# liyheng/MAGPO

Hardware: NVIDIA B200
Metric: end_to_end_training_agent_env_steps_per_sec (higher is better)
Workload: dtype f32

## Files before the change

### magpo_b200/csrc/retention_chunk.cu

```cuda
#include "common.cuh"
#include "kernels.cuh"

namespace magpo {
namespace {

constexpr int RC_ROWS = 32;
constexpr int LDA = 68;
constexpr int LDB = 72;
constexpr int LDP = 36;
constexpr int LDPT = 40;

struct Frag {
  uint32_t h[4], l[4];
};
struct FragB {
  uint32_t h[2], l[2];
};

__device__ __forceinline__ void split(float x, uint32_t& hi, uint32_t& lo) {
  hi = __float_as_uint(x) & 0xFFFFE000u;
  lo = __float_as_uint(x - __uint_as_float(hi));
}

__device__ __forceinline__ void mma8(float (&c)[4], const uint32_t (&a)[4], const uint32_t (&b)[2]) {
  asm volatile(
      "mma.sync.aligned.m16n8k8.row.col.f32.tf32.tf32.f32 {%0,%1,%2,%3}, {%4,%5,%6,%7}, {%8,%9}, {%0,%1,%2,%3};"
      : "+f"(c[0]), "+f"(c[1]), "+f"(c[2]), "+f"(c[3])
      : "r"(a[0]), "r"(a[1]), "r"(a[2]), "r"(a[3]), "r"(b[0]), "r"(b[1]));
}
__device__ __forceinline__ void mma3(float (&c)[4], const Frag& a, const FragB& b) {
  mma8(c, a.l, b.h);
  mma8(c, a.h, b.l);
  mma8(c, a.h, b.h);
}

__device__ __forceinline__ void ldsm_x4(const float* p, uint32_t (&r)[4]) {
  const uint32_t a = (uint32_t)__cvta_generic_to_shared(p);
  asm volatile("ldmatrix.sync.aligned.m8n8.x4.shared.b16 {%0,%1,%2,%3}, [%4];" : "=r"(r[0]), "=r"(r[1]), "=r"(r[2]), "=r"(r[3]) : "r"(a) : "memory");
}
__device__ __forceinline__ void ldsm_x2(const float* p, uint32_t (&r)[2]) {
  const uint32_t a = (uint32_t)__cvta_generic_to_shared(p);
  asm volatile("ldmatrix.sync.aligned.m8n8.x2.shared.b16 {%0,%1}, [%2];" : "=r"(r[0]), "=r"(r[1]) : "r"(a) : "memory");
}
__device__ __forceinline__ void split_u(uint32_t x, uint32_t& hi, uint32_t& lo) {
  hi = x & 0xFFFFE000u;
  lo = __float_as_uint(__uint_as_float(x) - __uint_as_float(hi));
}

__device__ __forceinline__ Frag lda_row(const float* X, int ld, int m0, int k0, int g, int tq) {
  const int lane = 4 * g + tq;
  uint32_t r[4];
  ldsm_x4(X + (m0 + (lane & 7) + ((lane >> 3) & 1) * 8) * ld + k0 + (lane >> 4) * 4, r);
  Frag f;
#pragma unroll
  for (int i = 0; i < 4; ++i) split_u(r[i], f.h[i], f.l[i]);
  return f;
}
__device__ __forceinline__ Frag lda_tr(const float* X, int ld, int m0, int k0, int g, int tq) {
  Frag f;
  split(X[(k0 + tq) * ld + m0 + g], f.h[0], f.l[0]);
  split(X[(k0 + tq) * ld + m0 + g + 8], f.h[1], f.l[1]);
  split(X[(k0 + tq + 4) * ld + m0 + g], f.h[2], f.l[2]);
  split(X[(k0 + tq + 4) * ld + m0 + g + 8], f.h[3], f.l[3]);
  return f;
}
__device__ __forceinline__ FragB ldb(const float* Y, int ld, int k0, int n0, int g, int tq) {
  FragB f;
  split(Y[(k0 + tq) * ld + n0 + g], f.h[0], f.l[0]);
  split(Y[(k0 + tq + 4) * ld + n0 + g], f.h[1], f.l[1]);
  return f;
}
__device__ __forceinline__ FragB ldb_tr(const float* Y, int ld, int k0, int n0, int g, int tq) {
  const int lane = 4 * g + tq;
  uint32_t r[2];
  ldsm_x2(Y + (n0 + (lane & 7)) * ld + k0 + ((lane >> 3) & 1) * 4, r);
  FragB f;
  split_u(r[0], f.h[0], f.l[0]);
  split_u(r[1], f.h[1], f.l[1]);
  return f;
}

__device__ __forceinline__ void zero4(float (&c)[4]) { c[0] = c[1] = c[2] = c[3] = 0.f; }

struct ChunkDecay {
  int cd_lane;
  __device__ __forceinline__ void init(const uint8_t* done, int t0, int L, int N, int n, int lane) {
    const bool d = done && lane < L && done[(int64_t)(t0 + lane) * N + n];
    const unsigned m = __ballot_sync(0xffffffffu, d);
    cd_lane = __popc(m & (0xffffffffu >> (31 - lane)));
  }
  __device__ __forceinline__ int cd(int tl) const { return __shfl_sync(0xffffffffu, cd_lane, tl); }
};

struct Tables {
  float* kpow;
  int* cds;
  uint8_t* row_tl;
};

template <bool CAUSAL>
__device__ __forceinline__ float decay_nm(const Tables& tb, int n, int m) {
  const int tn = tb.row_tl[n], tm = tb.row_tl[m];
  const bool order = CAUSAL ? (n >= m) : (tn >= tm);
  if (!order || tb.cds[tn] != tb.cds[tm]) return 0.f;
  return tb.kpow[tn - tm];
}

template <bool CAUSAL>
__global__ void __launch_bounds__(256, 2)
retention_chunk_fwd_kernel(int T, int N, int A, int Lc, float kappa, const float* __restrict__ q, const float* __restrict__ k,
                           const float* __restrict__ v, int ld, const float* __restrict__ H0, const uint8_t* __restrict__ done,
                           float* __restrict__ ret, float* __restrict__ Hck, float* __restrict__ Hout) {
  extern __shared__ __align__(16) float sm[];
  float* Hp = sm;
  float* Qs = Hp + 64 * LDB;
  float* Ks = Qs + RC_ROWS * LDA;
  float* Kt = Ks + RC_ROWS * LDA;
  float* Vs = Kt + RC_ROWS * LDB;
  float* Ps = Vs + RC_ROWS * LDB;
  Tables tb;
  tb.kpow = Ps + RC_ROWS * LDP;
  tb.cds = reinterpret_cast<int*>(tb.kpow + 40);
  tb.row_tl = reinterpret_cast<uint8_t*>(tb.cds + 32);

  const int n = blockIdx.x, tid = threadIdx.x, warp = tid >> 5, lane = tid & 31, g = lane >> 2, tq = lane & 3;
  if (tid == 0) {
    float p = 1.f;
    for (int j = 0; j < 40; ++j) { tb.kpow[j] = p; p *= kappa; }
  }
  if (tid < 32) tb.row_tl[tid] = (uint8_t)(tid / A);
  for (int i = tid; i < RC_ROWS * LDP; i += 256) Ps[i] = 0.f;

  const int mt = warp & 3, nt0 = (warp >> 2) * 4;
  float Hacc[4][4];
#pragma unroll
  for (int j = 0; j < 4; ++j) {
    const int r = 16 * mt + g, c = 8 * (nt0 + j) + 2 * tq;
    float2 lo2 = make_float2(0.f, 0.f), hi2 = make_float2(0.f, 0.f);
    if (H0) {
      lo2 = *reinterpret_cast<const float2*>(H0 + ((int64_t)n * 64 + r) * 64 + c);
      hi2 = *reinterpret_cast<const float2*>(H0 + ((int64_t)n * 64 + r + 8) * 64 + c);
    }
    Hacc[j][0] = lo2.x; Hacc[j][1] = lo2.y; Hacc[j][2] = hi2.x; Hacc[j][3] = hi2.y;
  }

  const int nchunks = (T + Lc - 1) / Lc;
  float pq[8], pk[8], pv[8];
  auto fetch = [&](int ch) {
    const int t0 = ch * Lc, L = min(Lc, T - t0), rows = L * A;
#pragma unroll
    for (int j = 0; j < 8; ++j) {
      const int idx = tid + j * 256, row = idx >> 6, col = idx & 63;
      pq[j] = pk[j] = pv[j] = 0.f;
      if (row < rows) {
        const int tl = tb.row_tl[row];
        const int64_t grow = ((int64_t)(t0 + tl) * N + n) * A + (row - tl * A);
        pq[j] = q[grow * ld + col]; pk[j] = k[grow * ld + col]; pv[j] = v[grow * ld + col];
      }
    }
  };
  __syncthreads();
  fetch(0);

  for (int ch = 0; ch < nchunks; ++ch) {
    const int t0 = ch * Lc, L = min(Lc, T - t0), rows = L * A;
    ChunkDecay cdk;
    cdk.init(done, t0, L, N, n, lane);
    const int cd_last = cdk.cd(L - 1);
    if (warp == 0) tb.cds[lane] = cdk.cd_lane;
#pragma unroll
    for (int j = 0; j < 4; ++j) {
      const int r = 16 * mt + g, c = 8 * (nt0 + j) + 2 * tq;
      *reinterpret_cast<float2*>(Hp + r * LDB + c) = make_float2(Hacc[j][0], Hacc[j][1]);
      *reinterpret_cast<float2*>(Hp + (r + 8) * LDB + c) = make_float2(Hacc[j][2], Hacc[j][3]);
      if (Hck) {
        float* dst = Hck + (((int64_t)ch * N + n) * 64) * 64;
        *reinterpret_cast<float2*>(dst + r * 64 + c) = make_float2(Hacc[j][0], Hacc[j][1]);
        *reinterpret_cast<float2*>(dst + (r + 8) * 64 + c) = make_float2(Hacc[j][2], Hacc[j][3]);
      }
    }
#pragma unroll
    for (int j = 0; j < 8; ++j) {
      const int idx = tid + j * 256, row = idx >> 6, col = idx & 63;
      const int tl = tb.row_tl[row];
      const int cdt = cdk.cd(tl);
      const float e = (row < rows && cdt == cd_last) ? tb.kpow[L - 1 - tl] : 0.f;
      Qs[row * LDA + col] = pq[j];
      Ks[row * LDA + col] = pk[j];
      Kt[row * LDB + col] = pk[j] * e;
      Vs[row * LDB + col] = pv[j];
    }
    __syncthreads();
    if (ch + 1 < nchunks) fetch(ch + 1);

    float o2[2][4];
    zero4(o2[0]); zero4(o2[1]);
    {
      const int mi = warp >> 2, ni = warp & 3;
      float s[4];
      zero4(s);
#pragma unroll
      for (int k0 = 0; k0 < 64; k0 += 8) {
        const Frag a0 = lda_row(Qs, LDA, 0, k0, g, tq);
        const Frag a1 = lda_row(Qs, LDA, 16, k0, g, tq);
        const FragB bk = ldb_tr(Ks, LDA, k0, 8 * ni, g, tq);
        mma3(s, mi ? a1 : a0, bk);
        const FragB bh = ldb(Hp, LDB, k0, 8 * warp, g, tq);
        mma3(o2[0], a0, bh);
        mma3(o2[1], a1, bh);
      }
      const int r = 16 * mi + g, c = 8 * ni + 2 * tq;
      Ps[r * LDP + c] = s[0] * decay_nm<CAUSAL>(tb, r, c);
      Ps[r * LDP + c + 1] = s[1] * decay_nm<CAUSAL>(tb, r, c + 1);
      Ps[(r + 8) * LDP + c] = s[2] * decay_nm<CAUSAL>(tb, r + 8, c);
      Ps[(r + 8) * LDP + c + 1] = s[3] * decay_nm<CAUSAL>(tb, r + 8, c + 1);
    }
    __syncthreads();

    {
      float o1[2][4];
      zero4(o1[0]); zero4(o1[1]);
#pragma unroll
      for (int k0 = 0; k0 < RC_ROWS; k0 += 8) {
        const FragB bv = ldb(Vs, LDB, k0, 8 * warp, g, tq);
        mma3(o1[0], lda_row(Ps, LDP, 0, k0, g, tq), bv);
        mma3(o1[1], lda_row(Ps, LDP, 16, k0, g, tq), bv);
      }
#pragma unroll
      for (int mi = 0; mi < 2; ++mi)
#pragma unroll
        for (int h = 0; h < 2; ++h) {
          const int row = 16 * mi + g + 8 * h;
          if (row < rows) {
            const int tl = tb.row_tl[row];
            const float cc = (tb.cds[tl] == 0) ? tb.kpow[tl + 1] : 0.f;
            const int64_t grow = ((int64_t)(t0 + tl) * N + n) * A + (row - tl * A);
            *reinterpret_cast<float2*>(ret + grow * 64 + 8 * warp + 2 * tq) =
                make_float2(o1[mi][2 * h] + cc * o2[mi][2 * h], o1[mi][2 * h + 1] + cc * o2[mi][2 * h + 1]);
          }
        }
    }
    {
      const float cL = (cd_last == 0) ? tb.kpow[L] : 0.f;
#pragma unroll
      for (int j = 0; j < 4; ++j)
#pragma unroll
        for (int x = 0; x < 4; ++x) Hacc[j][x] *= cL;
#pragma unroll
      for (int k0 = 0; k0 < RC_ROWS; k0 += 8) {
        const Frag a = lda_tr(Kt, LDB, 16 * mt, k0, g, tq);
#pragma unroll
        for (int j = 0; j < 4; ++j) mma3(Hacc[j], a, ldb(Vs, LDB, k0, 8 * (nt0 + j), g, tq));
      }
    }
    __syncthreads();
  }
  if (Hout) {
#pragma unroll
    for (int j = 0; j < 4; ++j) {
      const int r = 16 * mt + g, c = 8 * (nt0 + j) + 2 * tq;
      float* dst = Hout + (int64_t)n * 64 * 64;
      *reinterpret_cast<float2*>(dst + r * 64 + c) = make_float2(Hacc[j][0], Hacc[j][1]);
      *reinterpret_cast<float2*>(dst + (r + 8) * 64 + c) = make_float2(Hacc[j][2], Hacc[j][3]);
    }
  }
}

template <bool CAUSAL>
__global__ void __launch_bounds__(256, 2)
retention_chunk_bwd_kernel(int T, int N, int A, int Lc, float kappa, const float* __restrict__ q, const float* __restrict__ k,
                           const float* __restrict__ v, int ld, const uint8_t* __restrict__ done,
                           const float* __restrict__ Hck, const float* __restrict__ dret, float* __restrict__ dq,
                           float* __restrict__ dk, float* __restrict__ dv, int ldd) {
  extern __shared__ __align__(16) float sm[];
  float* Hp = sm;
  float* Gs = Hp + 64 * LDA;
  float* Gt = Gs + 64 * LDA;
  float* Qs = Gt + 64 * LDA;
  float* Ks = Qs + RC_ROWS * LDA;
  float* Vs = Ks + RC_ROWS * LDA;
  float* Ds = Vs + RC_ROWS * LDA;
  float* Qc = Ds + RC_ROWS * LDA;
  float* Ps = Qc + RC_ROWS * LDB;
  float* Ws = Ps + RC_ROWS * LDPT;
  Tables tb;
  tb.kpow = Ws + RC_ROWS * LDP;
  tb.cds = reinterpret_cast<int*>(tb.kpow + 40);
  tb.row_tl = reinterpret_cast<uint8_t*>(tb.cds + 32);

  const int n = blockIdx.x, tid = threadIdx.x, warp = tid >> 5, lane = tid & 31, g = lane >> 2, tq = lane & 3;
  if (tid == 0) {
    float p = 1.f;
    for (int j = 0; j < 40; ++j) { tb.kpow[j] = p; p *= kappa; }
  }
  if (tid < 32) tb.row_tl[tid] = (uint8_t)(tid / A);

  const int mt = warp & 3, nt0 = (warp >> 2) * 4;
  float Gacc[4][4];
#pragma unroll
  for (int j = 0; j < 4; ++j) zero4(Gacc[j]);

  const int nchunks = (T + Lc - 1) / Lc;
  float pq[8], pk[8], pv[8], pd[8];
  auto fetch = [&](int ch) {
    const int t0 = ch * Lc, L = min(Lc, T - t0), rows = L * A;
#pragma unroll
    for (int j = 0; j < 8; ++j) {
      const int idx = tid + j * 256, row = idx >> 6, col = idx & 63;
      pq[j] = pk[j] = pv[j] = pd[j] = 0.f;
      if (row < rows) {
        const int tl = tb.row_tl[row];
        const int64_t grow = ((int64_t)(t0 + tl) * N + n) * A + (row - tl * A);
        pq[j] = q[grow * ld + col]; pk[j] = k[grow * ld + col]; pv[j] = v[grow * ld + col];
        pd[j] = dret[grow * 64 + col];
      }
    }
  };
  __syncthreads();
  fetch(nchunks - 1);

  for (int ch = nchunks - 1; ch >= 0; --ch) {
    const int t0 = ch * Lc, L = min(Lc, T - t0), rows = L * A;
    ChunkDecay cdk;
    cdk.init(done, t0, L, N, n, lane);
    const int cd_last = cdk.cd(L - 1);
    if (warp == 0) tb.cds[lane] = cdk.cd_lane;
#pragma unroll
    for (int j = 0; j < 4; ++j) {
      const int r = 16 * mt + g, c = 8 * (nt0 + j) + 2 * tq;
      *reinterpret_cast<float2*>(Gs + r * LDA + c) = make_float2(Gacc[j][0], Gacc[j][1]);
      *reinterpret_cast<float2*>(Gs + (r + 8) * LDA + c) = make_float2(Gacc[j][2], Gacc[j][3]);
      Gt[c * LDA + r] = Gacc[j][0];
      Gt[(c + 1) * LDA + r] = Gacc[j][1];
      Gt[c * LDA + r + 8] = Gacc[j][2];
      Gt[(c + 1) * LDA + r + 8] = Gacc[j][3];
    }
    {
      const float4* src = reinterpret_cast<const float4*>(Hck + ((int64_t)ch * N + n) * 64 * 64);
#pragma unroll
      for (int j = 0; j < 4; ++j) {
        const int idx = tid + j * 256;
        const float4 h = src[idx];
        *reinterpret_cast<float4*>(Hp + (idx >> 4) * LDA + (idx & 15) * 4) = h;
      }
    }
#pragma unroll
    for (int j = 0; j < 8; ++j) {
      const int idx = tid + j * 256, row = idx >> 6, col = idx & 63;
      const int tl = tb.row_tl[row];
      const int cdt = cdk.cd(tl);
      const float cc = (row < rows && cdt == 0) ? tb.kpow[tl + 1] : 0.f;
      Qs[row * LDA + col] = pq[j];
      Ks[row * LDA + col] = pk[j];
      Vs[row * LDA + col] = pv[j];
      Ds[row * LDA + col] = pd[j];
      Qc[row * LDB + col] = pq[j] * cc;
    }
    __syncthreads();
    if (ch > 0) fetch(ch - 1);

    float dq2[2][4], dk2[2][4], dv2[2][4];
    zero4(dq2[0]); zero4(dq2[1]); zero4(dk2[0]); zero4(dk2[1]); zero4(dv2[0]); zero4(dv2[1]);
    {
      const int mi = warp >> 2, ni = warp & 3;
      float s[4], w[4];
      zero4(s); zero4(w);
#pragma unroll
      for (int k0 = 0; k0 < 64; k0 += 8) {
        {
          const Frag a = lda_row(Qs, LDA, 16 * mi, k0, g, tq);
          mma3(s, a, ldb_tr(Ks, LDA, k0, 8 * ni, g, tq));
        }
        const Frag d0 = lda_row(Ds, LDA, 0, k0, g, tq);
        const Frag d1 = lda_row(Ds, LDA, 16, k0, g, tq);
        mma3(w, mi ? d1 : d0, ldb_tr(Vs, LDA, k0, 8 * ni, g, tq));
        {
          const FragB b = ldb_tr(Hp, LDA, k0, 8 * warp, g, tq);
          mma3(dq2[0], d0, b);
          mma3(dq2[1], d1, b);
        }
        {
          const FragB b = ldb_tr(Gs, LDA, k0, 8 * warp, g, tq);
          mma3(dk2[0], lda_row(Vs, LDA, 0, k0, g, tq), b);
          mma3(dk2[1], lda_row(Vs, LDA, 16, k0, g, tq), b);
        }
        {
          const FragB b = ldb_tr(Gt, LDA, k0, 8 * warp, g, tq);
          mma3(dv2[0], lda_row(Ks, LDA, 0, k0, g, tq), b);
          mma3(dv2[1], lda_row(Ks, LDA, 16, k0, g, tq), b);
        }
      }
      const int r = 16 * mi + g, c = 8 * ni + 2 * tq;
      const float d00 = decay_nm<CAUSAL>(tb, r, c), d01 = decay_nm<CAUSAL>(tb, r, c + 1);
      const float d10 = decay_nm<CAUSAL>(tb, r + 8, c), d11 = decay_nm<CAUSAL>(tb, r + 8, c + 1);
      Ps[r * LDPT + c] = s[0] * d00; Ps[r * LDPT + c + 1] = s[1] * d01;
      Ps[(r + 8) * LDPT + c] = s[2] * d10; Ps[(r + 8) * LDPT + c + 1] = s[3] * d11;
      Ws[r * LDP + c] = w[0] * d00; Ws[r * LDP + c + 1] = w[1] * d01;
      Ws[(r + 8) * LDP + c] = w[2] * d10; Ws[(r + 8) * LDP + c + 1] = w[3] * d11;
    }
    __syncthreads();

    {
      float dq1[2][4], dk1[2][4], dv1[2][4];
      zero4(dq1[0]); zero4(dq1[1]); zero4(dk1[0]); zero4(dk1[1]); zero4(dv1[0]); zero4(dv1[1]);
#pragma unroll
      for (int k0 = 0; k0 < RC_ROWS; k0 += 8) {
        {
          const FragB b = ldb(Ks, LDA, k0, 8 * warp, g, tq);
          mma3(dq1[0], lda_row(Ws, LDP, 0, k0, g, tq), b);
          mma3(dq1[1], lda_row(Ws, LDP, 16, k0, g, tq), b);
        }
        {
          const FragB b = ldb(Qs, LDA, k0, 8 * warp, g, tq);
          mma3(dk1[0], lda_tr(Ws, LDP, 0, k0, g, tq), b);
          mma3(dk1[1], lda_tr(Ws, LDP, 16, k0, g, tq), b);
        }
        {
          const FragB b = ldb(Ds, LDA, k0, 8 * warp, g, tq);
          mma3(dv1[0], lda_tr(Ps, LDPT, 0, k0, g, tq), b);
          mma3(dv1[1], lda_tr(Ps, LDPT, 16, k0, g, tq), b);
        }
      }
#pragma unroll
      for (int mi = 0; mi < 2; ++mi)
#pragma unroll
        for (int h = 0; h < 2; ++h) {
          const int row = 16 * mi + g + 8 * h;
          if (row < rows) {
            const int tl = tb.row_tl[row];
            const int cdt = tb.cds[tl];
            const float cc = (cdt == 0) ? tb.kpow[tl + 1] : 0.f;
            const float ee = (cdt == cd_last) ? tb.kpow[L - 1 - tl] : 0.f;
            const int64_t grow = ((int64_t)(t0 + tl) * N + n) * A + (row - tl * A);
            const int col = 8 * warp + 2 * tq;
            *reinterpret_cast<float2*>(dq + grow * ldd + col) =
                make_float2(dq1[mi][2 * h] + cc * dq2[mi][2 * h], dq1[mi][2 * h + 1] + cc * dq2[mi][2 * h + 1]);
            *reinterpret_cast<float2*>(dk + grow * ldd + col) =
                make_float2(dk1[mi][2 * h] + ee * dk2[mi][2 * h], dk1[mi][2 * h + 1] + ee * dk2[mi][2 * h + 1]);
            *reinterpret_cast<float2*>(dv + grow * ldd + col) =
                make_float2(dv1[mi][2 * h] + ee * dv2[mi][2 * h], dv1[mi][2 * h + 1] + ee * dv2[mi][2 * h + 1]);
          }
        }
    }
    {
      const float cL = (cd_last == 0) ? tb.kpow[L] : 0.f;
#pragma unroll
      for (int j = 0; j < 4; ++j)
#pragma unroll
        for (int x = 0; x < 4; ++x) Gacc[j][x] *= cL;
#pragma unroll
      for (int k0 = 0; k0 < RC_ROWS; k0 += 8) {
        const Frag a = lda_tr(Qc, LDB, 16 * mt, k0, g, tq);
#pragma unroll
        for (int j = 0; j < 4; ++j) mma3(Gacc[j], a, ldb(Ds, LDA, k0, 8 * (nt0 + j), g, tq));
      }
    }
    __syncthreads();
  }
}

constexpr size_t kFwdSmem = (size_t)(64 * LDB + 2 * RC_ROWS * LDA + 2 * RC_ROWS * LDB + RC_ROWS * LDP + 40 + 32 + 8) * sizeof(float);
constexpr size_t kBwdSmem =
    (size_t)(3 * 64 * LDA + 4 * RC_ROWS * LDA + RC_ROWS * LDB + RC_ROWS * LDPT + RC_ROWS * LDP + 40 + 32 + 8) * sizeof(float);

template <typename Kern>
int set_smem(Kern kern, size_t bytes) {
  MAGPO_CUDA_OK(cudaFuncSetAttribute(kern, cudaFuncAttributeMaxDynamicSharedMemorySize, (int)bytes));
  return MAGPO_OK;
}

}

int retention_chunk_len(int A) { return std::max(1, RC_ROWS / A); }
int retention_num_chunks(int T, int A) { return (T + retention_chunk_len(A) - 1) / retention_chunk_len(A); }

int retention_chunk_fwd(cudaStream_t s, int T, int N, int A, float kappa, bool causal, const float* q, const float* k,
                        const float* v, int ld, const float* H0, const uint8_t* done, float* ret, float* Hck, float* Hout) {
  const int Lc = retention_chunk_len(A);
  if (once_per_device(ONCE_RET_FWD)) {
    MAGPO_TRY(set_smem(retention_chunk_fwd_kernel<true>, kFwdSmem));
    MAGPO_TRY(set_smem(retention_chunk_fwd_kernel<false>, kFwdSmem));
  }
  ProfScope ps(PROF_RET_FWD, s, 4.0 * 256.0 * (double)T * N * A);
  if (causal)
    retention_chunk_fwd_kernel<true><<<N, 256, kFwdSmem, s>>>(T, N, A, Lc, kappa, q, k, v, ld, H0, done, ret, Hck, Hout);
  else
    retention_chunk_fwd_kernel<false><<<N, 256, kFwdSmem, s>>>(T, N, A, Lc, kappa, q, k, v, ld, H0, done, ret, Hck, Hout);
  MAGPO_LAUNCH_OK();
  return MAGPO_OK;
}

int retention_chunk_bwd(cudaStream_t s, int T, int N, int A, float kappa, bool causal, const float* q, const float* k,
                        const float* v, int ld, const uint8_t* done, const float* Hck, const float* dret, float* dq,
                        float* dk, float* dv, int ldd) {
  const int Lc = retention_chunk_len(A);
  if (once_per_device(ONCE_RET_BWD)) {
    MAGPO_TRY(set_smem(retention_chunk_bwd_kernel<true>, kBwdSmem));
    MAGPO_TRY(set_smem(retention_chunk_bwd_kernel<false>, kBwdSmem));
  }
  ProfScope ps(PROF_RET_BWD, s, 7.0 * 256.0 * (double)T * N * A);
  if (causal)
    retention_chunk_bwd_kernel<true><<<N, 256, kBwdSmem, s>>>(T, N, A, Lc, kappa, q, k, v, ld, done, Hck, dret, dq, dk, dv, ldd);
  else
    retention_chunk_bwd_kernel<false><<<N, 256, kBwdSmem, s>>>(T, N, A, Lc, kappa, q, k, v, ld, done, Hck, dret, dq, dk, dv, ldd);
  MAGPO_LAUNCH_OK();
  return MAGPO_OK;
}

}
```

Baseline: 8.359 million.

## Prefetch chunk state via cp.async and hoist done-flag loads into fetch

In the backward retention kernel, the per-chunk Hck state load changes from synchronous float4 global reads into shared memory to cp.async issued one chunk ahead, right after the sync that follows Hp's last use. It is waited on at the start of the next iteration. The done-flag loads in both forward and backward kernels move into the prefetch lambda so their latency overlaps the previous chunk's compute. The aim is to hide global memory latency on the sequential chunk loop, which adds correctness risk around reuse of the Hp buffer.

```diff
diff --git a/magpo_b200/csrc/retention_chunk.cu b/magpo_b200/csrc/retention_chunk.cu
--- a/magpo_b200/csrc/retention_chunk.cu
+++ b/magpo_b200/csrc/retention_chunk.cu
@@ -80,12 +80,21 @@
   return f;
 }
 
+__device__ __forceinline__ void cp_async16(float* dst, const float* src) {
+  asm volatile("cp.async.cg.shared.global [%0], [%1], 16;" ::"r"((uint32_t)__cvta_generic_to_shared(dst)), "l"(src) : "memory");
+}
+__device__ __forceinline__ void cp_async_commit() { asm volatile("cp.async.commit_group;" ::: "memory"); }
+__device__ __forceinline__ void cp_async_wait_all() { asm volatile("cp.async.wait_all;" ::: "memory"); }
+
 __device__ __forceinline__ void zero4(float (&c)[4]) { c[0] = c[1] = c[2] = c[3] = 0.f; }
+
+__device__ __forceinline__ bool load_done(const uint8_t* done, int t0, int L, int N, int n, int lane) {
+  return done && lane < L && done[(int64_t)(t0 + lane) * N + n];
+}
 
 struct ChunkDecay {
   int cd_lane;
-  __device__ __forceinline__ void init(const uint8_t* done, int t0, int L, int N, int n, int lane) {
-    const bool d = done && lane < L && done[(int64_t)(t0 + lane) * N + n];
+  __device__ __forceinline__ void init(bool d, int lane) {
     const unsigned m = __ballot_sync(0xffffffffu, d);
     cd_lane = __popc(m & (0xffffffffu >> (31 - lane)));
   }
@@ -146,8 +155,10 @@
 
   const int nchunks = (T + Lc - 1) / Lc;
   float pq[8], pk[8], pv[8];
+  bool pdone;
   auto fetch = [&](int ch) {
     const int t0 = ch * Lc, L = min(Lc, T - t0), rows = L * A;
+    pdone = load_done(done, t0, L, N, n, lane);
 #pragma unroll
     for (int j = 0; j < 8; ++j) {
       const int idx = tid + j * 256, row = idx >> 6, col = idx & 63;
@@ -165,7 +176,7 @@
   for (int ch = 0; ch < nchunks; ++ch) {
     const int t0 = ch * Lc, L = min(Lc, T - t0), rows = L * A;
     ChunkDecay cdk;
-    cdk.init(done, t0, L, N, n, lane);
+    cdk.init(pdone, lane);
     const int cd_last = cdk.cd(L - 1);
     if (warp == 0) tb.cds[lane] = cdk.cd_lane;
 #pragma unroll
@@ -301,9 +312,20 @@
   for (int j = 0; j < 4; ++j) zero4(Gacc[j]);
 
   const int nchunks = (T + Lc - 1) / Lc;
+  auto load_state = [&](int ch) {
+    const float* src = Hck + ((int64_t)ch * N + n) * 64 * 64;
+#pragma unroll
+    for (int j = 0; j < 4; ++j) {
+      const int idx = tid + j * 256;
+      cp_async16(Hp + (idx >> 4) * LDA + (idx & 15) * 4, src + 4 * idx);
+    }
+    cp_async_commit();
+  };
   float pq[8], pk[8], pv[8], pd[8];
+  bool pdone;
   auto fetch = [&](int ch) {
     const int t0 = ch * Lc, L = min(Lc, T - t0), rows = L * A;
+    pdone = load_done(done, t0, L, N, n, lane);
 #pragma unroll
     for (int j = 0; j < 8; ++j) {
       const int idx = tid + j * 256, row = idx >> 6, col = idx & 63;
@@ -318,11 +340,12 @@
   };
   __syncthreads();
   fetch(nchunks - 1);
+  load_state(nchunks - 1);
 
   for (int ch = nchunks - 1; ch >= 0; --ch) {
     const int t0 = ch * Lc, L = min(Lc, T - t0), rows = L * A;
     ChunkDecay cdk;
-    cdk.init(done, t0, L, N, n, lane);
+    cdk.init(pdone, lane);
     const int cd_last = cdk.cd(L - 1);
     if (warp == 0) tb.cds[lane] = cdk.cd_lane;
 #pragma unroll
@@ -335,15 +358,7 @@
       Gt[c * LDA + r + 8] = Gacc[j][2];
       Gt[(c + 1) * LDA + r + 8] = Gacc[j][3];
     }
-    {
-      const float4* src = reinterpret_cast<const float4*>(Hck + ((int64_t)ch * N + n) * 64 * 64);
-#pragma unroll
-      for (int j = 0; j < 4; ++j) {
-        const int idx = tid + j * 256;
-        const float4 h = src[idx];
-        *reinterpret_cast<float4*>(Hp + (idx >> 4) * LDA + (idx & 15) * 4) = h;
-      }
-    }
+    cp_async_wait_all();
 #pragma unroll
     for (int j = 0; j < 8; ++j) {
       const int idx = tid + j * 256, row = idx >> 6, col = idx & 63;
@@ -399,6 +414,7 @@
       Ws[(r + 8) * LDP + c] = w[2] * d10; Ws[(r + 8) * LDP + c + 1] = w[3] * d11;
     }
     __syncthreads();
+    if (ch > 0) load_state(ch - 1);
 
     {
       float dq1[2][4], dk1[2][4], dv1[2][4];
```

After: 8.370 million (median of 6 runs). Within noise of the previous version (+0.1%).

## Restructure retention chunk kernels with pre-split transposed smem operands and async state prefetch

Applied to the files above, without the earlier changes.

Forward kernel now stores Q/K/Kt/V/P in shared memory already split into tf32 hi/lo halves and in transposed layouts, so every MMA operand is loaded with ldmatrix instead of scalar loads plus per-use splitting. The warp-to-tile mapping is changed so each warp reuses an A fragment across two N tiles, and the done-flag load is moved into the prefetch. The backward kernel keeps transposed copies (QcT, PT, WT) to replace strided lda_tr loads and prefetches the next chunk's Hck state with cp.async, overlapping it with compute. These changes use more shared memory, which may affect occupancy, and add extra stores per element.

```diff
diff --git a/magpo_b200/csrc/retention_chunk.cu b/magpo_b200/csrc/retention_chunk.cu
--- a/magpo_b200/csrc/retention_chunk.cu
+++ b/magpo_b200/csrc/retention_chunk.cu
@@ -6,9 +6,7 @@
 
 constexpr int RC_ROWS = 32;
 constexpr int LDA = 68;
-constexpr int LDB = 72;
 constexpr int LDP = 36;
-constexpr int LDPT = 40;
 
 struct Frag {
   uint32_t h[4], l[4];
@@ -54,14 +52,6 @@
   Frag f;
 #pragma unroll
   for (int i = 0; i < 4; ++i) split_u(r[i], f.h[i], f.l[i]);
-  return f;
-}
-__device__ __forceinline__ Frag lda_tr(const float* X, int ld, int m0, int k0, int g, int tq) {
-  Frag f;
-  split(X[(k0 + tq) * ld + m0 + g], f.h[0], f.l[0]);
-  split(X[(k0 + tq) * ld + m0 + g + 8], f.h[1], f.l[1]);
-  split(X[(k0 + tq + 4) * ld + m0 + g], f.h[2], f.l[2]);
-  split(X[(k0 + tq + 4) * ld + m0 + g + 8], f.h[3], f.l[3]);
   return f;
 }
 __device__ __forceinline__ FragB ldb(const float* Y, int ld, int k0, int n0, int g, int tq) {
@@ -82,10 +72,31 @@
 
 __device__ __forceinline__ void zero4(float (&c)[4]) { c[0] = c[1] = c[2] = c[3] = 0.f; }
 
+__device__ __forceinline__ void put_split(float* Xh, float* Xl, int i, float x) {
+  uint32_t hi, lo;
+  split(x, hi, lo);
+  Xh[i] = __uint_as_float(hi);
+  Xl[i] = __uint_as_float(lo);
+}
+__device__ __forceinline__ Frag lda_hl(const float* Xh, const float* Xl, int ld, int m0, int k0, int lane) {
+  const int off = (m0 + (lane & 7) + ((lane >> 3) & 1) * 8) * ld + k0 + (lane >> 4) * 4;
+  Frag f;
+  ldsm_x4(Xh + off, f.h);
+  ldsm_x4(Xl + off, f.l);
+  return f;
+}
+__device__ __forceinline__ FragB ldb_hl(const float* Yh, const float* Yl, int ld, int k0, int n0, int lane) {
+  const int off = (n0 + (lane & 7)) * ld + k0 + ((lane >> 3) & 1) * 4;
+  FragB f;
+  ldsm_x2(Yh + off, f.h);
+  ldsm_x2(Yl + off, f.l);
+  return f;
+}
+
+
 struct ChunkDecay {
   int cd_lane;
-  __device__ __forceinline__ void init(const uint8_t* done, int t0, int L, int N, int n, int lane) {
-    const bool d = done && lane < L && done[(int64_t)(t0 + lane) * N + n];
+  __device__ __forceinline__ void init(bool d, int lane) {
     const unsigned m = __ballot_sync(0xffffffffu, d);
     cd_lane = __popc(m & (0xffffffffu >> (31 - lane)));
   }
@@ -112,14 +123,19 @@
                            const float* __restrict__ v, int ld, const float* __restrict__ H0, const uint8_t* __restrict__ done,
                            float* __restrict__ ret, float* __restrict__ Hck, float* __restrict__ Hout) {
   extern __shared__ __align__(16) float sm[];
-  float* Hp = sm;
-  float* Qs = Hp + 64 * LDB;
-  float* Ks = Qs + RC_ROWS * LDA;
-  float* Kt = Ks + RC_ROWS * LDA;
-  float* Vs = Kt + RC_ROWS * LDB;
-  float* Ps = Vs + RC_ROWS * LDB;
+  float* HpT = sm;
+  float* Qh = HpT + 64 * LDA;
+  float* Ql = Qh + RC_ROWS * LDA;
+  float* Kh = Ql + RC_ROWS * LDA;
+  float* Kl = Kh + RC_ROWS * LDA;
+  float* KtTh = Kl + RC_ROWS * LDA;
+  float* KtTl = KtTh + 64 * LDP;
+  float* VTh = KtTl + 64 * LDP;
+  float* VTl = VTh + 64 * LDP;
+  float* Ph = VTl + 64 * LDP;
+  float* Pl = Ph + RC_ROWS * LDP;
   Tables tb;
-  tb.kpow = Ps + RC_ROWS * LDP;
+  tb.kpow = Pl + RC_ROWS * LDP;
   tb.cds = reinterpret_cast<int*>(tb.kpow + 40);
   tb.row_tl = reinterpret_cast<uint8_t*>(tb.cds + 32);
 
@@ -129,7 +145,6 @@
     for (int j = 0; j < 40; ++j) { tb.kpow[j] = p; p *= kappa; }
   }
   if (tid < 32) tb.row_tl[tid] = (uint8_t)(tid / A);
-  for (int i = tid; i < RC_ROWS * LDP; i += 256) Ps[i] = 0.f;
 
   const int mt = warp & 3, nt0 = (warp >> 2) * 4;
   float Hacc[4][4];
@@ -144,19 +159,20 @@
     Hacc[j][0] = lo2.x; Hacc[j][1] = lo2.y; Hacc[j][2] = hi2.x; Hacc[j][3] = hi2.y;
   }
 
+  const int op_row = 4 * warp + (lane & 3), op_col = lane >> 2;
   const int nchunks = (T + Lc - 1) / Lc;
   float pq[8], pk[8], pv[8];
+  bool pdone;
   auto fetch = [&](int ch) {
     const int t0 = ch * Lc, L = min(Lc, T - t0), rows = L * A;
+    pdone = done && lane < L && done[(int64_t)(t0 + lane) * N + n];
+    const int tl = op_row / A;
+    const int64_t grow = ((int64_t)(t0 + tl) * N + n) * A + (op_row - tl * A);
 #pragma unroll
     for (int j = 0; j < 8; ++j) {
-      const int idx = tid + j * 256, row = idx >> 6, col = idx & 63;
+      const int col = 8 * j + op_col;
       pq[j] = pk[j] = pv[j] = 0.f;
-      if (row < rows) {
-        const int tl = tb.row_tl[row];
-        const int64_t grow = ((int64_t)(t0 + tl) * N + n) * A + (row - tl * A);
-        pq[j] = q[grow * ld + col]; pk[j] = k[grow * ld + col]; pv[j] = v[grow * ld + col];
-      }
+      if (op_row < rows) { pq[j] = q[grow * ld + col]; pk[j] = k[grow * ld + col]; pv[j] = v[grow * ld + col]; }
     }
   };
   __syncthreads();
@@ -165,55 +181,56 @@
   for (int ch = 0; ch < nchunks; ++ch) {
     const int t0 = ch * Lc, L = min(Lc, T - t0), rows = L * A;
     ChunkDecay cdk;
-    cdk.init(done, t0, L, N, n, lane);
+    cdk.init(pdone, lane);
     const int cd_last = cdk.cd(L - 1);
     if (warp == 0) tb.cds[lane] = cdk.cd_lane;
 #pragma unroll
     for (int j = 0; j < 4; ++j) {
       const int r = 16 * mt + g, c = 8 * (nt0 + j) + 2 * tq;
-      *reinterpret_cast<float2*>(Hp + r * LDB + c) = make_float2(Hacc[j][0], Hacc[j][1]);
-      *reinterpret_cast<float2*>(Hp + (r + 8) * LDB + c) = make_float2(Hacc[j][2], Hacc[j][3]);
+      HpT[c * LDA + r] = Hacc[j][0];
+      HpT[(c + 1) * LDA + r] = Hacc[j][1];
+      HpT[c * LDA + r + 8] = Hacc[j][2];
+      HpT[(c + 1) * LDA + r + 8] = Hacc[j][3];
       if (Hck) {
         float* dst = Hck + (((int64_t)ch * N + n) * 64) * 64;
         *reinterpret_cast<float2*>(dst + r * 64 + c) = make_float2(Hacc[j][0], Hacc[j][1]);
         *reinterpret_cast<float2*>(dst + (r + 8) * 64 + c) = make_float2(Hacc[j][2], Hacc[j][3]);
       }
     }
-#pragma unroll
-    for (int j = 0; j < 8; ++j) {
-      const int idx = tid + j * 256, row = idx >> 6, col = idx & 63;
-      const int tl = tb.row_tl[row];
+    {
+      const int row = op_row, tl = tb.row_tl[row];
       const int cdt = cdk.cd(tl);
       const float e = (row < rows && cdt == cd_last) ? tb.kpow[L - 1 - tl] : 0.f;
-      Qs[row * LDA + col] = pq[j];
-      Ks[row * LDA + col] = pk[j];
-      Kt[row * LDB + col] = pk[j] * e;
-      Vs[row * LDB + col] = pv[j];
+#pragma unroll
+      for (int j = 0; j < 8; ++j) {
+        const int col = 8 * j + op_col;
+        put_split(Qh, Ql, row * LDA + col, pq[j]);
+        put_split(Kh, Kl, row * LDA + col, pk[j]);
+        put_split(KtTh, KtTl, col * LDP + row, pk[j] * e);
+        put_split(VTh, VTl, col * LDP + row, pv[j]);
+      }
     }
     __syncthreads();
     if (ch + 1 < nchunks) fetch(ch + 1);
 
+    const int mi = warp >> 2, ni = warp & 3;
     float o2[2][4];
     zero4(o2[0]); zero4(o2[1]);
     {
-      const int mi = warp >> 2, ni = warp & 3;
       float s[4];
       zero4(s);
 #pragma unroll
       for (int k0 = 0; k0 < 64; k0 += 8) {
-        const Frag a0 = lda_row(Qs, LDA, 0, k0, g, tq);
-        const Frag a1 = lda_row(Qs, LDA, 16, k0, g, tq);
-        const FragB bk = ldb_tr(Ks, LDA, k0, 8 * ni, g, tq);
-        mma3(s, mi ? a1 : a0, bk);
-        const FragB bh = ldb(Hp, LDB, k0, 8 * warp, g, tq);
-        mma3(o2[0], a0, bh);
-        mma3(o2[1], a1, bh);
+        const Frag a = lda_hl(Qh, Ql, LDA, 16 * mi, k0, lane);
+        mma3(s, a, ldb_hl(Kh, Kl, LDA, k0, 8 * ni, lane));
+        mma3(o2[0], a, ldb_tr(HpT, LDA, k0, 16 * ni, g, tq));
+        mma3(o2[1], a, ldb_tr(HpT, LDA, k0, 16 * ni + 8, g, tq));
       }
       const int r = 16 * mi + g, c = 8 * ni + 2 * tq;
-      Ps[r * LDP + c] = s[0] * decay_nm<CAUSAL>(tb, r, c);
-      Ps[r * LDP + c + 1] = s[1] * decay_nm<CAUSAL>(tb, r, c + 1);
-      Ps[(r + 8) * LDP + c] = s[2] * decay_nm<CAUSAL>(tb, r + 8, c);
-      Ps[(r + 8) * LDP + c + 1] = s[3] * decay_nm<CAUSAL>(tb, r + 8, c + 1);
+      put_split(Ph, Pl, r * LDP + c, s[0] * decay_nm<CAUSAL>(tb, r, c));
+      put_split(Ph, Pl, r * LDP + c + 1, s[1] * decay_nm<CAUSAL>(tb, r, c + 1));
+      put_split(Ph, Pl, (r + 8) * LDP + c, s[2] * decay_nm<CAUSAL>(tb, r + 8, c));
+      put_split(Ph, Pl, (r + 8) * LDP + c + 1, s[3] * decay_nm<CAUSAL>(tb, r + 8, c + 1));
     }
     __syncthreads();
 
@@ -222,23 +239,23 @@
       zero4(o1[0]); zero4(o1[1]);
 #pragma unroll
       for (int k0 = 0; k0 < RC_ROWS; k0 += 8) {
-        const FragB bv = ldb(Vs, LDB, k0, 8 * warp, g, tq);
-        mma3(o1[0], lda_row(Ps, LDP, 0, k0, g, tq), bv);
-        mma3(o1[1], lda_row(Ps, LDP, 16, k0, g, tq), bv);
-      }
-#pragma unroll
-      for (int mi = 0; mi < 2; ++mi)
-#pragma unroll
-        for (int h = 0; h < 2; ++h) {
-          const int row = 16 * mi + g + 8 * h;
-          if (row < rows) {
-            const int tl = tb.row_tl[row];
-            const float cc = (tb.cds[tl] == 0) ? tb.kpow[tl + 1] : 0.f;
-            const int64_t grow = ((int64_t)(t0 + tl) * N + n) * A + (row - tl * A);
-            *reinterpret_cast<float2*>(ret + grow * 64 + 8 * warp + 2 * tq) =
-                make_float2(o1[mi][2 * h] + cc * o2[mi][2 * h], o1[mi][2 * h + 1] + cc * o2[mi][2 * h + 1]);
-          }
-        }
+        const Frag a = lda_hl(Ph, Pl, LDP, 16 * mi, k0, lane);
+        mma3(o1[0], a, ldb_hl(VTh, VTl, LDP, k0, 16 * ni, lane));
+        mma3(o1[1], a, ldb_hl(VTh, VTl, LDP, k0, 16 * ni + 8, lane));
+      }
+#pragma unroll
+      for (int h = 0; h < 2; ++h) {
+        const int row = 16 * mi + g + 8 * h;
+        if (row < rows) {
+          const int tl = tb.row_tl[row];
+          const float cc = (tb.cds[tl] == 0) ? tb.kpow[tl + 1] : 0.f;
+          const int64_t grow = ((int64_t)(t0 + tl) * N + n) * A + (row - tl * A);
+#pragma unroll
+          for (int jj = 0; jj < 2; ++jj)
+            *reinterpret_cast<float2*>(ret + grow * 64 + 16 * ni + 8 * jj + 2 * tq) =
+                make_float2(o1[jj][2 * h] + cc * o2[jj][2 * h], o1[jj][2 * h + 1] + cc * o2[jj][2 * h + 1]);
+        }
+      }
     }
     {
       const float cL = (cd_last == 0) ? tb.kpow[L] : 0.f;
@@ -248,9 +265,9 @@
         for (int x = 0; x < 4; ++x) Hacc[j][x] *= cL;
 #pragma unroll
       for (int k0 = 0; k0 < RC_ROWS; k0 += 8) {
-        const Frag a = lda_tr(Kt, LDB, 16 * mt, k0, g, tq);
-#pragma unroll
-        for (int j = 0; j < 4; ++j) mma3(Hacc[j], a, ldb(Vs, LDB, k0, 8 * (nt0 + j), g, tq));
+        const Frag a = lda_hl(KtTh, KtTl, LDP, 16 * mt, k0, lane);
+#pragma unroll
+        for (int j = 0; j < 4; ++j) mma3(Hacc[j], a, ldb_hl(VTh, VTl, LDP, k0, 8 * (nt0 + j), lane));
       }
     }
     __syncthreads();
@@ -265,6 +282,11 @@
     }
   }
 }
+
+__device__ __forceinline__ void cp_async16(float* dst, const float* src) {
+  asm volatile("cp.async.cg.shared.global [%0], [%1], 16;" ::"r"((uint32_t)__cvta_generic_to_shared(dst)), "l"(src) : "memory");
+}
+__device__ __forceinline__ void cp_async_wait_all() { asm volatile("cp.async.wait_all;" ::: "memory"); }
 
 template <bool CAUSAL>
 __global__ void __launch_bounds__(256, 2)
@@ -280,11 +302,12 @@
   float* Ks = Qs + RC_ROWS * LDA;
   float* Vs = Ks + RC_ROWS * LDA;
   float* Ds = Vs + RC_ROWS * LDA;
-  float* Qc = Ds + RC_ROWS * LDA;
-  float* Ps = Qc + RC_ROWS * LDB;
-  float* Ws = Ps + RC_ROWS * LDPT;
+  float* QcT = Ds + RC_ROWS * LDA;
+  float* PT = QcT + 64 * LDP;
+  float* Ws = PT + RC_ROWS * LDP;
+  float* WT = Ws + RC_ROWS * LDP;
   Tables tb;
-  tb.kpow = Ws + RC_ROWS * LDP;
+  tb.kpow = WT + RC_ROWS * LDP;
   tb.cds = reinterpret_cast<int*>(tb.kpow + 40);
   tb.row_tl = reinterpret_cast<uint8_t*>(tb.cds + 32);
 
@@ -300,29 +323,41 @@
 #pragma unroll
   for (int j = 0; j < 4; ++j) zero4(Gacc[j]);
 
+  auto fetch_state = [&](int ch) {
+    const float* src = Hck + ((int64_t)ch * N + n) * 64 * 64;
+#pragma unroll
+    for (int j = 0; j < 4; ++j) {
+      const int idx = tid + j * 256;
+      cp_async16(Hp + (idx >> 4) * LDA + (idx & 15) * 4, src + idx * 4);
+    }
+  };
+  const int op_row = 4 * warp + (lane & 3), op_col = lane >> 2;
   const int nchunks = (T + Lc - 1) / Lc;
   float pq[8], pk[8], pv[8], pd[8];
+  bool pdone;
   auto fetch = [&](int ch) {
     const int t0 = ch * Lc, L = min(Lc, T - t0), rows = L * A;
+    pdone = done && lane < L && done[(int64_t)(t0 + lane) * N + n];
+    const int tl = op_row / A;
+    const int64_t grow = ((int64_t)(t0 + tl) * N + n) * A + (op_row - tl * A);
 #pragma unroll
     for (int j = 0; j < 8; ++j) {
-      const int idx = tid + j * 256, row = idx >> 6, col = idx & 63;
+      const int col = 8 * j + op_col;
       pq[j] = pk[j] = pv[j] = pd[j] = 0.f;
-      if (row < rows) {
-        const int tl = tb.row_tl[row];
-        const int64_t grow = ((int64_t)(t0 + tl) * N + n) * A + (row - tl * A);
+      if (op_row < rows) {
         pq[j] = q[grow * ld + col]; pk[j] = k[grow * ld + col]; pv[j] = v[grow * ld + col];
         pd[j] = dret[grow * 64 + col];
       }
     }
   };
   __syncthreads();
+  fetch_state(nchunks - 1);
   fetch(nchunks - 1);
 
   for (int ch = nchunks - 1; ch >= 0; --ch) {
     const int t0 = ch * Lc, L = min(Lc, T - t0), rows = L * A;
     ChunkDecay cdk;
-    cdk.init(done, t0, L, N, n, lane);
+    cdk.init(pdone, lane);
     const int cd_last = cdk.cd(L - 1);
     if (warp == 0) tb.cds[lane] = cdk.cd_lane;
 #pragma unroll
@@ -336,69 +371,61 @@
       Gt[(c + 1) * LDA + r + 8] = Gacc[j][3];
     }
     {
-      const float4* src = reinterpret_cast<const float4*>(Hck + ((int64_t)ch * N + n) * 64 * 64);
-#pragma unroll
-      for (int j = 0; j < 4; ++j) {
-        const int idx = tid + j * 256;
-        const float4 h = src[idx];
-        *reinterpret_cast<float4*>(Hp + (idx >> 4) * LDA + (idx & 15) * 4) = h;
-      }
-    }
-#pragma unroll
-    for (int j = 0; j < 8; ++j) {
-      const int idx = tid + j * 256, row = idx >> 6, col = idx & 63;
-      const int tl = tb.row_tl[row];
+      const int row = op_row, tl = tb.row_tl[row];
       const int cdt = cdk.cd(tl);
       const float cc = (row < rows && cdt == 0) ? tb.kpow[tl + 1] : 0.f;
-      Qs[row * LDA + col] = pq[j];
-      Ks[row * LDA + col] = pk[j];
-      Vs[row * LDA + col] = pv[j];
-      Ds[row * LDA + col] = pd[j];
-      Qc[row * LDB + col] = pq[j] * cc;
-    }
+#pragma unroll
+      for (int j = 0; j < 8; ++j) {
+        const int col = 8 * j + op_col;
+        Qs[row * LDA + col] = pq[j];
+        Ks[row * LDA + col] = pk[j];
+        Vs[row * LDA + col] = pv[j];
+        Ds[row * LDA + col] = pd[j];
+        QcT[col * LDP + row] = pq[j] * cc;
+      }
+    }
+    cp_async_wait_all();
     __syncthreads();
     if (ch > 0) fetch(ch - 1);
 
+    const int mi = warp >> 2, cg = warp & 3;
     float dq2[2][4], dk2[2][4], dv2[2][4];
     zero4(dq2[0]); zero4(dq2[1]); zero4(dk2[0]); zero4(dk2[1]); zero4(dv2[0]); zero4(dv2[1]);
     {
-      const int mi = warp >> 2, ni = warp & 3;
       float s[4], w[4];
       zero4(s); zero4(w);
 #pragma unroll
       for (int k0 = 0; k0 < 64; k0 += 8) {
+        mma3(s, lda_row(Qs, LDA, 16 * mi, k0, g, tq), ldb_tr(Ks, LDA, k0, 8 * cg, g, tq));
+        const Frag d = lda_row(Ds, LDA, 16 * mi, k0, g, tq);
+        mma3(w, d, ldb_tr(Vs, LDA, k0, 8 * cg, g, tq));
+#pragma unroll
+        for (int jj = 0; jj < 2; ++jj)
+          mma3(dq2[jj], d, ldb_tr(Hp, LDA, k0, 16 * cg + 8 * jj, g, tq));
         {
-          const Frag a = lda_row(Qs, LDA, 16 * mi, k0, g, tq);
-          mma3(s, a, ldb_tr(Ks, LDA, k0, 8 * ni, g, tq));
-        }
-        const Frag d0 = lda_row(Ds, LDA, 0, k0, g, tq);
-        const Frag d1 = lda_row(Ds, LDA, 16, k0, g, tq);
-        mma3(w, mi ? d1 : d0, ldb_tr(Vs, LDA, k0, 8 * ni, g, tq));
+          const Frag a = lda_row(Vs, LDA, 16 * mi, k0, g, tq);
+#pragma unroll
+          for (int jj = 0; jj < 2; ++jj) mma3(dk2[jj], a, ldb_tr(Gs, LDA, k0, 16 * cg + 8 * jj, g, tq));
+        }
         {
-          const FragB b = ldb_tr(Hp, LDA, k0, 8 * warp, g, tq);
-          mma3(dq2[0], d0, b);
-          mma3(dq2[1], d1, b);
-        }
-        {
-          const FragB b = ldb_tr(Gs, LDA, k0, 8 * warp, g, tq);
-          mma3(dk2[0], lda_row(Vs, LDA, 0, k0, g, tq), b);
-          mma3(dk2[1], lda_row(Vs, LDA, 16, k0, g, tq), b);
-        }
-        {
-          const FragB b = ldb_tr(Gt, LDA, k0, 8 * warp, g, tq);
-          mma3(dv2[0], lda_row(Ks, LDA, 0, k0, g, tq), b);
-          mma3(dv2[1], lda_row(Ks, LDA, 16, k0, g, tq), b);
-        }
-      }
-      const int r = 16 * mi + g, c = 8 * ni + 2 * tq;
+          const Frag a = lda_row(Ks, LDA, 16 * mi, k0, g, tq);
+#pragma unroll
+          for (int jj = 0; jj < 2; ++jj) mma3(dv2[jj], a, ldb_tr(Gt, LDA, k0, 16 * cg + 8 * jj, g, tq));
+        }
+      }
+      const int r = 16 * mi + g, c = 8 * cg + 2 * tq;
       const float d00 = decay_nm<CAUSAL>(tb, r, c), d01 = decay_nm<CAUSAL>(tb, r, c + 1);
       const float d10 = decay_nm<CAUSAL>(tb, r + 8, c), d11 = decay_nm<CAUSAL>(tb, r + 8, c + 1);
-      Ps[r * LDPT + c] = s[0] * d00; Ps[r * LDPT + c + 1] = s[1] * d01;
-      Ps[(r + 8) * LDPT + c] = s[2] * d10; Ps[(r + 8) * LDPT + c + 1] = s[3] * d11;
-      Ws[r * LDP + c] = w[0] * d00; Ws[r * LDP + c + 1] = w[1] * d01;
-      Ws[(r + 8) * LDP + c] = w[2] * d10; Ws[(r + 8) * LDP + c + 1] = w[3] * d11;
+      PT[c * LDP + r] = s[0] * d00; PT[(c + 1) * LDP + r] = s[1] * d01;
+      PT[c * LDP + r + 8] = s[2] * d10; PT[(c + 1) * LDP + r + 8] = s[3] * d11;
+      const float w00 = w[0] * d00, w01 = w[1] * d01, w10 = w[2] * d10, w11 = w[3] * d11;
+      Ws[r * LDP + c] = w00; Ws[r * LDP + c + 1] = w01;
+      Ws[(r + 8) * LDP + c] = w10; Ws[(r + 8) * LDP + c + 1] = w11;
+      WT[c * LDP + r] = w00; WT[(c + 1) * LDP + r] = w01;
+      WT[c * LDP + r + 8] = w10; WT[(c + 1) * LDP + r + 8] = w11;
     }
     __syncthreads();
+    if (ch > 0) fetch_state(ch - 1);
 
     {
       float dq1[2][4], dk1[2][4], dv1[2][4];
@@ -406,41 +433,42 @@
 #pragma unroll
       for (int k0 = 0; k0 < RC_ROWS; k0 += 8) {
         {
-          const FragB b = ldb(Ks, LDA, k0, 8 * warp, g, tq);
-          mma3(dq1[0], lda_row(Ws, LDP, 0, k0, g, tq), b);
-          mma3(dq1[1], lda_row(Ws, LDP, 16, k0, g, tq), b);
+          const Frag a = lda_row(Ws, LDP, 16 * mi, k0, g, tq);
+#pragma unroll
+          for (int jj = 0; jj < 2; ++jj) mma3(dq1[jj], a, ldb(Ks, LDA, k0, 16 * cg + 8 * jj, g, tq));
         }
         {
-          const FragB b = ldb(Qs, LDA, k0, 8 * warp, g, tq);
-          mma3(dk1[0], lda_tr(Ws, LDP, 0, k0, g, tq), b);
-          mma3(dk1[1], lda_tr(Ws, LDP, 16, k0, g, tq), b);
+          const Frag a = lda_row(WT, LDP, 16 * mi, k0, g, tq);
+#pragma unroll
+          for (int jj = 0; jj < 2; ++jj) mma3(dk1[jj], a, ldb(Qs, LDA, k0, 16 * cg + 8 * jj, g, tq));
         }
         {
-          const FragB b = ldb(Ds, LDA, k0, 8 * warp, g, tq);
-          mma3(dv1[0], lda_tr(Ps, LDPT, 0, k0, g, tq), b);
-          mma3(dv1[1], lda_tr(Ps, LDPT, 16, k0, g, tq), b);
-        }
-      }
-#pragma unroll
-      for (int mi = 0; mi < 2; ++mi)
-#pragma unroll
-        for (int h = 0; h < 2; ++h) {
-          const int row = 16 * mi + g + 8 * h;
-          if (row < rows) {
-            const int tl = tb.row_tl[row];
-            const int cdt = tb.cds[tl];
-            const float cc = (cdt == 0) ? tb.kpow[tl + 1] : 0.f;
-            const float ee = (cdt == cd_last) ? tb.kpow[L - 1 - tl] : 0.f;
-            const int64_t grow = ((int64_t)(t0 + tl) * N + n) * A + (row - tl * A);
-            const int col = 8 * warp + 2 * tq;
+          const Frag a = lda_row(PT, LDP, 16 * mi, k0, g, tq);
+#pragma unroll
+          for (int jj = 0; jj < 2; ++jj) mma3(dv1[jj], a, ldb(Ds, LDA, k0, 16 * cg + 8 * jj, g, tq));
+        }
+      }
+#pragma unroll
+      for (int h = 0; h < 2; ++h) {
+        const int row = 16 * mi + g + 8 * h;
+        if (row < rows) {
+          const int tl = tb.row_tl[row];
+          const int cdt = tb.cds[tl];
+          const float cc = (cdt == 0) ? tb.kpow[tl + 1] : 0.f;
+          const float ee = (cdt == cd_last) ? tb.kpow[L - 1 - tl] : 0.f;
+          const int64_t grow = ((int64_t)(t0 + tl) * N + n) * A + (row - tl * A);
+#pragma unroll
+          for (int jj = 0; jj < 2; ++jj) {
+            const int col = 16 * cg + 8 * jj + 2 * tq;
             *reinterpret_cast<float2*>(dq + grow * ldd + col) =
-                make_float2(dq1[mi][2 * h] + cc * dq2[mi][2 * h], dq1[mi][2 * h + 1] + cc * dq2[mi][2 * h + 1]);
+                make_float2(dq1[jj][2 * h] + cc * dq2[jj][2 * h], dq1[jj][2 * h + 1] + cc * dq2[jj][2 * h + 1]);
             *reinterpret_cast<float2*>(dk + grow * ldd + col) =
-                make_float2(dk1[mi][2 * h] + ee * dk2[mi][2 * h], dk1[mi][2 * h + 1] + ee * dk2[mi][2 * h + 1]);
+                make_float2(dk1[jj][2 * h] + ee * dk2[jj][2 * h], dk1[jj][2 * h + 1] + ee * dk2[jj][2 * h + 1]);
             *reinterpret_cast<float2*>(dv + grow * ldd + col) =
-                make_float2(dv1[mi][2 * h] + ee * dv2[mi][2 * h], dv1[mi][2 * h + 1] + ee * dv2[mi][2 * h + 1]);
+                make_float2(dv1[jj][2 * h] + ee * dv2[jj][2 * h], dv1[jj][2 * h + 1] + ee * dv2[jj][2 * h + 1]);
           }
         }
+      }
     }
     {
       const float cL = (cd_last == 0) ? tb.kpow[L] : 0.f;
@@ -450,7 +478,7 @@
         for (int x = 0; x < 4; ++x) Gacc[j][x] *= cL;
 #pragma unroll
       for (int k0 = 0; k0 < RC_ROWS; k0 += 8) {
-        const Frag a = lda_tr(Qc, LDB, 16 * mt, k0, g, tq);
+        const Frag a = lda_row(QcT, LDP, 16 * mt, k0, g, tq);
 #pragma unroll
         for (int j = 0; j < 4; ++j) mma3(Gacc[j], a, ldb(Ds, LDA, k0, 8 * (nt0 + j), g, tq));
       }
@@ -459,9 +487,9 @@
   }
 }
 
-constexpr size_t kFwdSmem = (size_t)(64 * LDB + 2 * RC_ROWS * LDA + 2 * RC_ROWS * LDB + RC_ROWS * LDP + 40 + 32 + 8) * sizeof(float);
+constexpr size_t kFwdSmem = (size_t)(64 * LDA + 4 * RC_ROWS * LDA + 4 * 64 * LDP + 2 * RC_ROWS * LDP + 40 + 32 + 8) * sizeof(float);
 constexpr size_t kBwdSmem =
-    (size_t)(3 * 64 * LDA + 4 * RC_ROWS * LDA + RC_ROWS * LDB + RC_ROWS * LDPT + RC_ROWS * LDP + 40 + 32 + 8) * sizeof(float);
+    (size_t)(3 * 64 * LDA + 4 * RC_ROWS * LDA + 64 * LDP + 3 * RC_ROWS * LDP + 40 + 32 + 8) * sizeof(float);
 
 template <typename Kern>
 int set_smem(Kern kern, size_t bytes) {
```

Result: no change. 8.474 million before, 8.534 million after, median of 6 (+0.7%).
